# quantumjot/sequitr

Measured on AMD Instinct MI355X. Metric: segmented Mpixels/sec on 512x512 tiles; IoU vs reference, higher is better.
Workload: dtype f32; 1 GPU; U-Net 2-class inference, launches of 32 512x512x1 tiles, fp32 (BASELINE.json configs[1]: filters 16-32-64-128-256, eltwise_mul bridge); logits + uint8 argmax mask; one 32-tile batch per GPU per step; tiles_this_rank=32

## Files before the change

sequitr_amd/csrc/sq_common.h:

```cpp
#pragma once
#include <hip/hip_runtime.h>
#include <stdint.h>
#include <stdio.h>
#include "../../include/sequitr_hip.h"

typedef float f32x4 __attribute__((ext_vector_type(4)));

#define SQ_NOT_MINE 1

void sq_set_error(const char *fmt, ...);

#define SQ_REQUIRE(cond, ...)            \
    do {                                 \
        if (!(cond)) {                   \
            sq_set_error(__VA_ARGS__);   \
            return SQ_EINVAL;            \
        }                                \
    } while (0)

int sq_plan_bf16_kc(int Cin);
int sq_plan_bf16_bn(int64_t ntiles, int Cout, bool pn, bool mos);
int sq_plan_mosaic_splitk(int Nimg, int h, int w, int Cin, int Cout, int R, int Cc, bool have_ws, int64_t workspace_bytes);
int sq_plan_f32_bn(int64_t ntiles, int Cout);
bool sq_plan_f32_stage32(int bn, int KS, int KC, int Cin, bool concat);
bool sq_plan_l0_takes(int mode, int cout, int act, int H, int W, bool concat, int head_c, bool pooled);
int sq_wgrad_f32_plan(int N, int H, int W, int Cin, int Cout, int K, int64_t *out);

#define SQ_ALIGNED16(p) ((((uintptr_t)(p)) & 15u) == 0)

#define SQ_REQUIRE_ALIGNED(p)                                     \
    do {                                                          \
        if (!SQ_ALIGNED16(p)) {                                   \
            sq_set_error("%s: pointer %s not 16-byte aligned", __func__, #p); \
            return SQ_EALIGN;                                     \
        }                                                         \
    } while (0)

static inline int sq_check_launch(const char *what) {
    hipError_t e = hipGetLastError();
    if (e != hipSuccess) {
        sq_set_error("%s: launch failed: %s", what, hipGetErrorString(e));
        return SQ_ELAUNCH;
    }
    return SQ_OK;
}

__device__ __forceinline__ float sq_act(float v, int act) {
    if (act == SQ_ACT_RELU) return v > 0.0f ? v : 0.0f;
    if (act == SQ_ACT_LEAKY) return v > 0.0f ? v : 0.2f * v;
    return v;
}

__device__ __forceinline__ unsigned sq_xcd_remap(unsigned bid, unsigned nblk) {
    const unsigned q = nblk >> 3, r = nblk & 7u, xcd = bid & 7u, k = bid >> 3;
    const unsigned base = xcd < r ? xcd * (q + 1) : r * (q + 1) + (xcd - r) * q;
    return base + k;
}

struct SqDropKey { unsigned s1, s2; };
__device__ __forceinline__ SqDropKey sq_dropout_key(unsigned seed, const int *__restrict__ step) {
    if (step) seed += (unsigned)step[0] * 0x9E3779B9u;
    SqDropKey k;
    k.s1 = seed * 0x9E3779B1u + 0x7F4A7C15u;
    k.s2 = (seed ^ 0x68E31DA4u) * 0x85EBCA6Bu;
    k.s2 ^= k.s2 >> 13;
    return k;
}
__device__ __forceinline__ unsigned sq_dropout_thr16(float rate) { return (unsigned)(rate * 65536.0f); }
__device__ __forceinline__ unsigned sq_dropout_keep4(SqDropKey k, unsigned q, unsigned thr16) {
    unsigned h = q + k.s1;
    h ^= h >> 16; h *= 0x7FEB352Du; h = h ^ (h >> 15) ^ k.s2; h *= 0x846CA68Bu; h ^= h >> 16;
    unsigned g = (h ^ 0x5BD1E995u) * 0x2C1B3C6Du;
    g ^= g >> 15;
    return (unsigned)((h & 0xFFFFu) >= thr16) | ((unsigned)((h >> 16) >= thr16) << 1) |
           ((unsigned)((g & 0xFFFFu) >= thr16) << 2) | ((unsigned)((g >> 16) >= thr16) << 3);
}

template <int MAXC>
__device__ __forceinline__ float sq_wce_pixel(const float (&zc)[MAXC], const float (&yc)[MAXC], int C, float wp, float g,
                                              float *__restrict__ dz) {
#pragma clang fp contract(off)
    float m = -INFINITY, yt = 0.f, dot = 0.f;
#pragma unroll
    for (int c = 0; c < MAXC; ++c)
        if (c < C) {
            m = zc[c] > m ? zc[c] : m;
            yt += yc[c];
            dot = __builtin_fmaf(yc[c], zc[c], dot);
        }
    float s = 0.f;
#pragma unroll
    for (int c = 0; c < MAXC; ++c)
        if (c < C) s += expf(zc[c] - m);
    const float lse = m + logf(s);
    if (dz) {
#pragma unroll
        for (int c = 0; c < MAXC; ++c)
            if (c < C) dz[c] = g * (expf(zc[c] - lse) * yt - yc[c]);
    }
    return wp * (lse * yt - dot);
}

__device__ __forceinline__ float sq_group_reduce(const float *__restrict__ p, size_t stride, int nblk, int g, int G) {
    float s = 0.f;
    int b = g;
    for (; b + 7 * G < nblk; b += 8 * G) {
        float v[8];
#pragma unroll
        for (int u = 0; u < 8; ++u) v[u] = p[(size_t)(b + u * G) * stride];
#pragma unroll
        for (int u = 0; u < 8; ++u) s += v[u];
    }
    for (; b < nblk; b += G) s += p[(size_t)b * stride];
    for (int m = G >> 1; m > 0; m >>= 1) s += __shfl_xor(s, m);
    return s;
}
static inline int sq_group_size(int nblk) {
    int G = 1;
    while (G < 64 && G * 2 <= nblk) G *= 2;
    return G;
}
```

sequitr_amd/csrc/sq_conv_f32_l0.hip:

```cpp
#include <stdlib.h>
#include "sq_common.h"
#include "sq_conv_epi.h"

#ifndef SQ_L0_SETPRIO
#define SQ_L0_SETPRIO 1
#endif
#ifndef SQ_L0_OCC
#define SQ_L0_OCC 4
#endif
#ifndef SQ_L0_UP_OCC
#define SQ_L0_UP_OCC 2
#endif

namespace {

constexpr int TH = 16, TW = 16, HWD = 18, HP = HWD * HWD;
constexpr int PS = 24;
constexpr int XS_FLOATS = HP * PS;
constexpr int XITEMS = HP * 4, XSLOTS = 6;
constexpr int IN_W = 20, IN_FLOATS = IN_W * IN_W;
constexpr int UP_W = 10, UP_CIN = 32, UP_PS = 40, UP_FLOATS = UP_W * UP_W * UP_PS;
constexpr unsigned OOB = 0x80000000u;

enum { EPI_STORE = 0, EPI_POOL = 1, EPI_HEAD = 2 };
enum { M_PLAIN = 0, M_FIRST = 1, M_UP = 2 };

struct L0Args {
    const float *x, *w, *bias;
    float *y;
    int N, H, W;
    int tiles_x, tiles_y, ntiles;
    int gx, gy, gn;
    SqConvEpi epi;
};

struct Pos { int tx, ty, n; };

typedef unsigned u32x4 __attribute__((__vector_size__(4 * sizeof(unsigned))));
typedef unsigned u32x2 __attribute__((__vector_size__(2 * sizeof(unsigned))));

__device__ __forceinline__ void row_transpose(float &a0, float &a1, float &a2, float &a3) {
    const auto p = __builtin_amdgcn_permlane16_swap(__float_as_uint(a0), __float_as_uint(a1), false, false);
    const auto q = __builtin_amdgcn_permlane16_swap(__float_as_uint(a2), __float_as_uint(a3), false, false);
    const auto u = __builtin_amdgcn_permlane32_swap(p[0], q[0], false, false);
    const auto v = __builtin_amdgcn_permlane32_swap(p[1], q[1], false, false);
    a0 = __uint_as_float(u[0]); a2 = __uint_as_float(u[1]);
    a1 = __uint_as_float(v[0]); a3 = __uint_as_float(v[1]);
}

__device__ __forceinline__ float relu(float v) { return __builtin_fmaxf(v, 0.0f); }

template <int MODE, int EPI, int BRIDGE, int NB>
__global__ __launch_bounds__(256, (MODE == M_UP ? SQ_L0_UP_OCC : (NB == 2 ? 2 : SQ_L0_OCC))) void conv_l0_kernel(const L0Args a) {
    static_assert(NB == 1 || (NB == 2 && MODE == M_PLAIN && EPI == EPI_STORE), "32 output channels: the plain form only");
    constexpr int CO = 16 * NB;
    extern __shared__ __attribute__((aligned(16))) float smem[];
    float *xs = smem;
    float *xin = smem + XS_FLOATS;
    float *xl = smem + XS_FLOATS;

    const int tid = threadIdx.x, lane = tid & 63, wv = tid >> 6;
    const int li = lane & 15, kk = lane >> 4;
    const int H = a.H, W = a.W;
    const int G = (int)gridDim.x;
    const int vb = (int)sq_xcd_remap(blockIdx.x, gridDim.x);
    if (vb >= a.ntiles) return;
    const int t_count = (a.ntiles - vb + G - 1) / G;

    const __amdgpu_buffer_rsrc_t xrsrc = __builtin_amdgcn_make_buffer_rsrc(
        const_cast<float *>(a.x), 0, (int)((size_t)a.N * H * W * (MODE == M_FIRST ? 1 : 16) * 4), 0x00020000);
    const __amdgpu_buffer_rsrc_t yrsrc = __builtin_amdgcn_make_buffer_rsrc(
        a.y, 0, a.y ? (int)((size_t)a.N * H * W * CO * 4) : 0, 0x00020000);

    float af[9][4][NB];
#pragma unroll
    for (int t = 0; t < 9; ++t)
#pragma unroll
        for (int s = 0; s < 4; ++s)
#pragma unroll
            for (int nb = 0; nb < NB; ++nb) af[t][s][nb] = a.w[(t * 16 + 4 * s + kk) * CO + nb * 16 + li];
    float4 bv[NB];
#pragma unroll
    for (int nb = 0; nb < NB; ++nb)
        bv[nb] = a.bias ? *reinterpret_cast<const float4 *>(a.bias + nb * 16 + 4 * kk) : make_float4(0.f, 0.f, 0.f, 0.f);

    auto decode = [&](int tile) {
        Pos p;
        p.tx = tile % a.tiles_x;
        p.ty = (tile / a.tiles_x) % a.tiles_y;
        p.n = tile / (a.tiles_x * a.tiles_y);
        return p;
    };
    auto advance = [&](Pos p) {
        p.tx += a.gx;
        if (p.tx >= a.tiles_x) { p.tx -= a.tiles_x; p.ty += 1; }
        p.ty += a.gy;
        if (p.ty >= a.tiles_y) { p.ty -= a.tiles_y; p.n += 1; }
        p.n += a.gn;
        return p;
    };
    auto interior = [&](const Pos &p) {
        return p.tx > 0 && p.tx < a.tiles_x - 1 && p.ty > 0 && p.ty < a.tiles_y - 1;
    };

    float4 xr[XSLOTS];
    int xrel[XSLOTS], xpp[XSLOTS];
    if constexpr (MODE == M_PLAIN) {
#pragma unroll
        for (int sl = 0; sl < XSLOTS; ++sl) {
            const int idx = tid + sl * 256, pix = idx >> 2, q = idx & 3;
            const int py = pix / HWD, px = pix % HWD;
            xrel[sl] = idx < XITEMS ? ((py * W + px) * 16 + q * 4) * 4 : (int)OOB;
            xpp[sl] = (py << 8) | px;
        }
    }
    auto issue_halo = [&](const Pos &p) {
        const int x0 = p.tx * TW - 1, y0 = p.ty * TH - 1;
        const int base = (((p.n * H + y0) * W + x0) * 16) * 4;
        if (interior(p)) {
#pragma unroll
            for (int sl = 0; sl < XSLOTS; ++sl) {
                const auto v = __builtin_amdgcn_raw_buffer_load_b128(xrsrc, xrel[sl], base, 0);
                xr[sl] = *reinterpret_cast<const float4 *>(&v);
            }
        } else {
#pragma unroll
            for (int sl = 0; sl < XSLOTS; ++sl) {
                const int py = xpp[sl] >> 8, px = xpp[sl] & 255;
                const bool inb = (unsigned)(y0 + py) < (unsigned)H && (unsigned)(x0 + px) < (unsigned)W && xrel[sl] != (int)OOB;
                const unsigned off = inb ? (unsigned)(base + xrel[sl]) : OOB;
                const auto v = __builtin_amdgcn_raw_buffer_load_b128(xrsrc, off, 0, 0);
                xr[sl] = *reinterpret_cast<const float4 *>(&v);
            }
        }
    };
    float *cw = xs + (tid >> 2) * PS + (tid & 3);
    auto commit_halo = [&]() {
#pragma unroll
        for (int sl = 0; sl < XSLOTS; ++sl) {
            if (sl < XSLOTS - 1 || tid < XITEMS - (XSLOTS - 1) * 256) {
                float *d = cw + sl * 64 * PS;
                d[0] = xr[sl].x; d[4] = xr[sl].y; d[8] = xr[sl].z; d[12] = xr[sl].w;
            }
        }
    };

    float a1[3] = {0.f, 0.f, 0.f};
    int toff[3] = {0, 0, 0};
    float4 b1v = make_float4(0.f, 0.f, 0.f, 0.f);
    float inr[2] = {0.f, 0.f};
    int fsrc[6] = {0, 0, 0, 0, 0, 0}, fpix[6] = {0, 0, 0, 0, 0, 0};
    int irel[2] = {0, 0};
    if constexpr (MODE == M_FIRST) {
#pragma unroll
        for (int s = 0; s < 3; ++s) {
            const int tap = 4 * s + kk;
            a1[s] = tap < 9 ? a.epi.first_w[tap * 16 + li] : 0.f;
            const int tc = tap < 9 ? tap : 8;
            toff[s] = (tc / 3) * IN_W + tc % 3;
        }
        b1v = *reinterpret_cast<const float4 *>(a.epi.first_b + 4 * kk);
#pragma unroll
        for (int i = 0; i < 6; ++i) {
            const int pix = (wv + 4 * i) * 16 + li, pc = pix < HP ? pix : HP - 1;
            fsrc[i] = (pc / HWD) * IN_W + pc % HWD;
            fpix[i] = pix;
        }
#pragma unroll
        for (int sl = 0; sl < 2; ++sl) {
            const int idx = tid + sl * 256;
            irel[sl] = idx < IN_FLOATS ? ((idx / IN_W) * W + idx % IN_W) * 4 : (int)OOB;
        }
    }
    auto issue_patch = [&](const Pos &p) {
        const int x0 = p.tx * TW - 2, y0 = p.ty * TH - 2;
        const int base = ((p.n * H + y0) * W + x0) * 4;
        if (interior(p)) {
#pragma unroll
            for (int sl = 0; sl < 2; ++sl)
                inr[sl] = __builtin_bit_cast(float, __builtin_amdgcn_raw_buffer_load_b32(xrsrc, irel[sl], base, 0));
        } else {
#pragma unroll
            for (int sl = 0; sl < 2; ++sl) {
                const int idx = tid + sl * 256, py = idx / IN_W, px = idx % IN_W;
                const bool inb = idx < IN_FLOATS && (unsigned)(y0 + py) < (unsigned)H && (unsigned)(x0 + px) < (unsigned)W;
                const unsigned off = inb ? (unsigned)(base + irel[sl]) : OOB;
                inr[sl] = __builtin_bit_cast(float, __builtin_amdgcn_raw_buffer_load_b32(xrsrc, off, 0, 0));
            }
        }
    };
    auto commit_patch = [&](int buf) {
        float *d = xin + buf * IN_FLOATS;
        d[tid] = inr[0];
        if (tid < IN_FLOATS - 256) d[tid + 256] = inr[1];
    };
    auto first_conv = [&](const Pos &p, int buf) {
        const float *src = xin + buf * IN_FLOATS;
        const bool inner = interior(p);
#pragma unroll
        for (int i = 0; i < 6; ++i) {
            if (wv + 4 * i < (HP + 15) / 16) {
                f32x4 c1 = (f32x4){0.f, 0.f, 0.f, 0.f};
#pragma unroll
                for (int s = 0; s < 3; ++s)
                    c1 = __builtin_amdgcn_mfma_f32_16x16x4f32(a1[s], src[fsrc[i] + toff[s]], c1, 0, 0, 0);
                float v0 = relu(c1[0] + b1v.x), v1 = relu(c1[1] + b1v.y), v2 = relu(c1[2] + b1v.z), v3 = relu(c1[3] + b1v.w);
                if (!inner) {
                    const int pc = fpix[i] < HP ? fpix[i] : HP - 1;
                    const int gy = p.ty * TH - 1 + pc / HWD, gx = p.tx * TW - 1 + pc % HWD;
                    const bool inside = (unsigned)gy < (unsigned)H && (unsigned)gx < (unsigned)W;
                    v0 = inside ? v0 : 0.f; v1 = inside ? v1 : 0.f; v2 = inside ? v2 : 0.f; v3 = inside ? v3 : 0.f;
                }
                row_transpose(v0, v1, v2, v3);
                if (fpix[i] < HP) *reinterpret_cast<float4 *>(xs + fpix[i] * PS + 4 * kk) = make_float4(v0, v1, v2, v3);
            }
        }
    };

    float aw[8] = {0.f, 0.f, 0.f, 0.f, 0.f, 0.f, 0.f, 0.f};
    float4 upb = make_float4(0.f, 0.f, 0.f, 0.f);
    float4 lr[4], sr[6];
    int srel[6] = {0, 0, 0, 0, 0, 0}, lrel[4] = {0, 0, 0, 0};
    unsigned upk[6] = {0, 0, 0, 0, 0, 0};
    const int Hl = H >> 1, Wl = W >> 1;
    const __amdgpu_buffer_rsrc_t lrsrc = __builtin_amdgcn_make_buffer_rsrc(
        const_cast<float *>(a.epi.up_x), 0, MODE == M_UP ? (int)((size_t)a.N * Hl * Wl * UP_CIN * 4) : 0, 0x00020000);
    if constexpr (MODE == M_UP) {
#pragma unroll
        for (int s8 = 0; s8 < 8; ++s8) aw[s8] = a.epi.up_w[(wv * 16 + li) * UP_CIN + 4 * s8 + kk];
        if (a.epi.up_b) upb = *reinterpret_cast<const float4 *>(a.epi.up_b + 4 * kk);
        const int oy = ((wv >> 1) + 1) & 1, ox = ((wv & 1) + 1) & 1;
#pragma unroll
        for (int blk = 0; blk < 6; ++blk) {
            const int j = blk * 16 + li, jc = j < 81 ? j : 80;
            const int hy = 2 * (jc / 9) + oy, hx = 2 * (jc % 9) + ox;
            srel[blk] = j < 81 ? ((hy * W + hx) * 16 + 4 * kk) * 4 : (int)OOB;
            const unsigned usrc = (((hy + 1) >> 1) * UP_W + ((hx + 1) >> 1)) * UP_PS + 4 * kk;
            const unsigned udst = j < 81 ? (hy * HWD + hx) * PS + 4 * kk : 0xFFFFu;
            upk[blk] = usrc | (udst << 16);
        }
#pragma unroll
        for (int sl = 0; sl < 4; ++sl) {
            const int idx = tid + sl * 256, lp = idx >> 3, q = idx & 7;
            lrel[sl] = idx < UP_W * UP_W * 8 ? (((lp / UP_W) * Wl + lp % UP_W) * UP_CIN + q * 4) * 4 : (int)OOB;
        }
    }
    auto issue_skip = [&](const Pos &p) {
        const int x0 = p.tx * TW - 1, y0 = p.ty * TH - 1;
        const int base = (((p.n * H + y0) * W + x0) * 16) * 4;
        if (interior(p)) {
#pragma unroll
            for (int blk = 0; blk < 6; ++blk) {
                const auto v = __builtin_amdgcn_raw_buffer_load_b128(xrsrc, srel[blk], base, 0);
                sr[blk] = *reinterpret_cast<const float4 *>(&v);
            }
        } else {
            const int oy = ((wv >> 1) + 1) & 1, ox = ((wv & 1) + 1) & 1;
#pragma unroll
            for (int blk = 0; blk < 6; ++blk) {
                const int j = blk * 16 + li, jc = j < 81 ? j : 80;
                const int hy = 2 * (jc / 9) + oy, hx = 2 * (jc % 9) + ox;
                const bool inb = j < 81 && (unsigned)(y0 + hy) < (unsigned)H && (unsigned)(x0 + hx) < (unsigned)W;
                const unsigned off = inb ? (unsigned)(base + srel[blk]) : OOB;
                const auto v = __builtin_amdgcn_raw_buffer_load_b128(xrsrc, off, 0, 0);
                sr[blk] = *reinterpret_cast<const float4 *>(&v);
            }
        }
    };
    auto issue_low = [&](const Pos &p) {
        const int ly0 = p.ty * (TH / 2) - 1, lx0 = p.tx * (TW / 2) - 1;
        const int base = (((p.n * Hl + ly0) * Wl + lx0) * UP_CIN) * 4;
        if (interior(p)) {
#pragma unroll
            for (int sl = 0; sl < 4; ++sl) {
                const auto v = __builtin_amdgcn_raw_buffer_load_b128(lrsrc, lrel[sl], base, 0);
                lr[sl] = *reinterpret_cast<const float4 *>(&v);
            }
        } else {
#pragma unroll
            for (int sl = 0; sl < 4; ++sl) {
                const int idx = tid + sl * 256, lp = idx >> 3;
                const int ly = lp / UP_W, lx = lp % UP_W;
                const bool inb = idx < UP_W * UP_W * 8 && (unsigned)(ly0 + ly) < (unsigned)Hl && (unsigned)(lx0 + lx) < (unsigned)Wl;
                const unsigned off = inb ? (unsigned)(base + lrel[sl]) : OOB;
                const auto v = __builtin_amdgcn_raw_buffer_load_b128(lrsrc, off, 0, 0);
                lr[sl] = *reinterpret_cast<const float4 *>(&v);
            }
        }
    };
    float *lw = xl + (tid >> 3) * UP_PS + ((tid & 7) >> 2) * 16 + (tid & 3);
    auto commit_low = [&]() {
#pragma unroll
        for (int sl = 0; sl < 4; ++sl) {
            if (sl < 3 || tid < UP_W * UP_W * 8 - 768) {
                float *d = lw + sl * 32 * UP_PS;
                d[0] = lr[sl].x; d[4] = lr[sl].y; d[8] = lr[sl].z; d[12] = lr[sl].w;
            }
        }
    };
    auto up_conv = [&](const Pos &p) {
        const bool inner = interior(p);
#pragma unroll
        for (int bp = 0; bp < 6; bp += 2) {
            float4 bl[2][2];
#pragma unroll
            for (int t = 0; t < 2; ++t) {
                const float *src = xl + (upk[bp + t] & 0xFFFFu);
                bl[t][0] = *reinterpret_cast<const float4 *>(src);
                bl[t][1] = *reinterpret_cast<const float4 *>(src + 16);
            }
            f32x4 c1[2];
#pragma unroll
            for (int s8 = 0; s8 < 8; ++s8) {
#pragma unroll
                for (int t = 0; t < 2; ++t) {
                    const float4 q = bl[t][s8 >> 2];
                    const float b = (s8 & 3) == 0 ? q.x : ((s8 & 3) == 1 ? q.y : ((s8 & 3) == 2 ? q.z : q.w));
                    c1[t] = __builtin_amdgcn_mfma_f32_16x16x4f32(aw[s8], b, s8 == 0 ? (f32x4){0.f, 0.f, 0.f, 0.f} : c1[t], 0, 0, 0);
                }
            }
#pragma unroll
            for (int t = 0; t < 2; ++t) {
                const int blk = bp + t;
                const float u[4] = {c1[t][0] + upb.x, c1[t][1] + upb.y, c1[t][2] + upb.z, c1[t][3] + upb.w};
                const float sk[4] = {sr[blk].x, sr[blk].y, sr[blk].z, sr[blk].w};
                float m[4];
#pragma unroll
                for (int e = 0; e < 4; ++e)
                    m[e] = BRIDGE == SQ_BRIDGE_ADD ? u[e] + sk[e]
                         : (BRIDGE == SQ_BRIDGE_MUL ? u[e] * sk[e] : (BRIDGE == SQ_BRIDGE_SUB ? u[e] - sk[e] : u[e]));
                if (!inner) {
                    const int j = blk * 16 + li, jc = j < 81 ? j : 80;
                    const int hy = 2 * (jc / 9) + (((wv >> 1) + 1) & 1), hx = 2 * (jc % 9) + (((wv & 1) + 1) & 1);
                    const int gy = p.ty * TH - 1 + hy, gx = p.tx * TW - 1 + hx;
                    const bool inside = (unsigned)gy < (unsigned)H && (unsigned)gx < (unsigned)W;
#pragma unroll
                    for (int e = 0; e < 4; ++e) m[e] = inside ? m[e] : 0.f;
                }
                row_transpose(m[0], m[1], m[2], m[3]);
                if ((upk[blk] >> 16) != 0xFFFFu) *reinterpret_cast<float4 *>(xs + (upk[blk] >> 16)) = make_float4(m[0], m[1], m[2], m[3]);
            }
        }
    };

    f32x4 acc[4][NB];
    const float *xb = xs + ((4 * wv) * HWD + li) * PS + 4 * kk;
    auto mfma_phase = [&]() {
        float4 bq[2][3];
#pragma unroll
        for (int kx = 0; kx < 3; ++kx) bq[0][kx] = *reinterpret_cast<const float4 *>(xb + kx * PS);
#if SQ_L0_SETPRIO
        __builtin_amdgcn_s_setprio(0);
#endif
#pragma unroll
        for (int h = 0; h < 6; ++h) {
            if (h + 1 < 6) {
#pragma unroll
                for (int kx = 0; kx < 3; ++kx)
                    bq[(h + 1) & 1][kx] = *reinterpret_cast<const float4 *>(xb + ((h + 1) * HWD + kx) * PS);
            }
            __builtin_amdgcn_sched_barrier(0);
#pragma unroll
            for (int kx = 0; kx < 3; ++kx) {
                const float4 q = bq[h & 1][kx];
                const float b[4] = {q.x, q.y, q.z, q.w};
#pragma unroll
                for (int s = 0; s < 4; ++s) {
#pragma unroll
                    for (int ky = 2; ky >= 0; --ky) {
                        const int r = h - ky;
                        if (r < 0 || r > 3) continue;
                        const bool first = ky == 0 && kx == 0 && s == 0;
#pragma unroll
                        for (int nb = 0; nb < NB; ++nb)
                            acc[r][nb] = __builtin_amdgcn_mfma_f32_16x16x4f32(af[ky * 3 + kx][s][nb], b[s],
                                                                              first ? (f32x4){0.f, 0.f, 0.f, 0.f} : acc[r][nb], 0, 0, 0);
                    }
                }
            }
            __builtin_amdgcn_sched_barrier(0);
        }
#if SQ_L0_SETPRIO
        __builtin_amdgcn_s_setprio(3);
#endif
    };

    const int yvoff = (((4 * wv) * W + li) * CO + 4 * kk) * 4;
    const __amdgpu_buffer_rsrc_t prsrc = __builtin_amdgcn_make_buffer_rsrc(
        a.epi.pooled, 0, EPI == EPI_POOL ? (int)((size_t)a.N * Hl * Wl * 16 * 4) : 0, 0x00020000);
    const int pvoff = (((2 * wv) * Wl + (li >> 1)) * 16 + 4 * kk) * 4;
    float *hws = smem + XS_FLOATS;
    float hb0 = 0.f, hb1 = 0.f;
    const __amdgpu_buffer_rsrc_t grsrc = __builtin_amdgcn_make_buffer_rsrc(
        a.epi.logits, 0, EPI == EPI_HEAD ? (int)((size_t)a.N * H * W * 2 * 4) : 0, 0x00020000);
    const __amdgpu_buffer_rsrc_t mrsrc = __builtin_amdgcn_make_buffer_rsrc(
        a.epi.mask, 0, (EPI == EPI_HEAD && a.epi.mask) ? (int)((size_t)a.N * H * W) : 0, 0x00020000);
    const int gvoff = ((4 * wv + kk) * W + li) * 8, mvoff = (4 * wv + kk) * W + li;
    if constexpr (EPI == EPI_HEAD) {
        static_assert(MODE == M_PLAIN, "the head table sits right behind the halo image");
        if (tid < 64) hws[tid] = (tid >> 4) < 2 ? a.epi.head_w[(tid & 15) * 2 + (tid >> 4)] : 0.f;
        if (a.epi.head_b) { hb0 = a.epi.head_b[0]; hb1 = a.epi.head_b[1]; }
    }
    auto epilogue = [&](const Pos &p) {
        if constexpr (NB > 1) {
            const int tbase = (((p.n * H + p.ty * TH) * W + p.tx * TW) * CO) * 4;
#pragma unroll
            for (int r = 0; r < 4; ++r)
#pragma unroll
                for (int nb = 0; nb < NB; ++nb) {
                    const f32x4 t = (f32x4){relu(acc[r][nb][0] + bv[nb].x), relu(acc[r][nb][1] + bv[nb].y),
                                            relu(acc[r][nb][2] + bv[nb].z), relu(acc[r][nb][3] + bv[nb].w)};
                    __builtin_amdgcn_raw_buffer_store_b128(*reinterpret_cast<const u32x4 *>(&t), yrsrc,
                                                           yvoff + tbase + r * W * CO * 4 + nb * 64, 0, 0);
                }
            return;
        }
        float o[4][4];
#pragma unroll
        for (int r = 0; r < 4; ++r) {
            o[r][0] = relu(acc[r][0][0] + bv[0].x); o[r][1] = relu(acc[r][0][1] + bv[0].y);
            o[r][2] = relu(acc[r][0][2] + bv[0].z); o[r][3] = relu(acc[r][0][3] + bv[0].w);
        }
        if constexpr (EPI != EPI_HEAD) {
            const int tbase = (((p.n * H + p.ty * TH) * W + p.tx * TW) * 16) * 4;
#pragma unroll
            for (int r = 0; r < 4; ++r) {
                const f32x4 t = (f32x4){o[r][0], o[r][1], o[r][2], o[r][3]};
                __builtin_amdgcn_raw_buffer_store_b128(*reinterpret_cast<const u32x4 *>(&t), yrsrc, yvoff + tbase + r * W * 64, 0, 0);
            }
        }
        if constexpr (EPI == EPI_POOL) {
            const int pbase = (((p.n * Hl + p.ty * (TH / 2)) * Wl + p.tx * (TW / 2)) * 16) * 4;
#pragma unroll
            for (int pr = 0; pr < 2; ++pr) {
                f32x4 mp;
#pragma unroll
                for (int j = 0; j < 4; ++j) {
                    const float v = __builtin_fmaxf(o[2 * pr][j], o[2 * pr + 1][j]);
                    const float u = __builtin_bit_cast(float, __builtin_amdgcn_mov_dpp(__builtin_bit_cast(int, v), 0xB1, 0xF, 0xF, true));
                    mp[j] = __builtin_fmaxf(u, v);
                }
                __builtin_amdgcn_raw_buffer_store_b128(*reinterpret_cast<const u32x4 *>(&mp), prsrc,
                                                       (li & 1) ? (int)OOB : pvoff + pbase + pr * Wl * 64, 0, 0);
            }
        }
        if constexpr (EPI == EPI_HEAD) {
#pragma unroll
            for (int j = 0; j < 4; ++j) row_transpose(o[0][j], o[1][j], o[2][j], o[3][j]);
            float4 hq[4];
#pragma unroll
            for (int r = 0; r < 4; ++r) hq[r] = *reinterpret_cast<const float4 *>(hws + (lane & 3) * 16 + 4 * r);
            f32x4 z = (f32x4){0.f, 0.f, 0.f, 0.f};
#pragma unroll
            for (int r = 0; r < 4; ++r) {
                const float hv[4] = {hq[r].x, hq[r].y, hq[r].z, hq[r].w};
#pragma unroll
                for (int j = 0; j < 4; ++j) z = __builtin_amdgcn_mfma_f32_4x4x1f32(hv[j], o[r][j], z, 0, 0, 0);
            }
            const float z0 = z[0], z1 = z[1];
            const float v0 = a.epi.head_b ? z0 + hb0 : z0, v1 = a.epi.head_b ? z1 + hb1 : z1;
            const int pbase = (p.n * H + p.ty * TH) * W + p.tx * TW;
            const float lg[2] = {v0, v1};
            __builtin_amdgcn_raw_buffer_store_b64(*reinterpret_cast<const u32x2 *>(lg), grsrc, gvoff, pbase * 8, 0);
            __builtin_amdgcn_raw_buffer_store_b8((unsigned char)(v1 > v0 ? 1 : 0), mrsrc, mvoff, pbase, 0);
        }
    };

    Pos cur = decode(vb), nxt = cur, nn = cur;
    if constexpr (MODE == M_PLAIN) {
        issue_halo(cur);
        __builtin_amdgcn_s_waitcnt(0x0F70);
        commit_halo();
        __syncthreads();
        for (int it = 0; it < t_count; ++it) {
            const bool has_next = it + 1 < t_count;
            if (has_next) { nxt = advance(cur); issue_halo(nxt); }
            mfma_phase();
            __builtin_amdgcn_s_waitcnt(0x0F70);
            if (has_next) {
                __syncthreads();
                commit_halo();
            }
            epilogue(cur);
            if (has_next) __syncthreads();
            cur = nxt;
        }
    }
    if constexpr (MODE == M_FIRST) {
        issue_patch(cur);
        __builtin_amdgcn_s_waitcnt(0x0F70);
        commit_patch(0);
        __syncthreads();
        first_conv(cur, 0);
        if (t_count > 1) {
            nxt = advance(cur);
            issue_patch(nxt);
            __builtin_amdgcn_s_waitcnt(0x0F70);
            commit_patch(1);
        }
        __syncthreads();
        for (int it = 0; it < t_count; ++it) {
            const bool has_next = it + 1 < t_count, has_next2 = it + 2 < t_count;
            if (has_next2) { nn = advance(nxt); issue_patch(nn); }
            mfma_phase();
            __builtin_amdgcn_s_waitcnt(0x0F70);
            if (has_next) {
                __syncthreads();
                first_conv(nxt, (it + 1) & 1);
            }
            if (has_next2) commit_patch(it & 1);
            epilogue(cur);
            if (has_next) __syncthreads();
            cur = nxt;
            nxt = nn;
        }
    }
    if constexpr (MODE == M_UP) {
        issue_low(cur);
        issue_skip(cur);
        __builtin_amdgcn_s_waitcnt(0x0F70);
        commit_low();
        if (t_count > 1) { nxt = advance(cur); issue_low(nxt); }
        __syncthreads();
        up_conv(cur);
        __builtin_amdgcn_s_waitcnt(0x0F70);
        __syncthreads();
        for (int it = 0; it < t_count; ++it) {
            const bool has_next = it + 1 < t_count, has_next2 = it + 2 < t_count;
            if (has_next) { commit_low(); issue_skip(nxt); }
            if (has_next2) { nn = advance(nxt); issue_low(nn); }
            mfma_phase();
            __builtin_amdgcn_s_waitcnt(0x0F70);
            if (has_next) {
                __syncthreads();
                up_conv(nxt);
            }
            epilogue(cur);
            if (has_next) __syncthreads();
            cur = nxt;
            nxt = nn;
        }
    }
}

template <int MODE, int EPI, int BRIDGE = 0, int NB = 1>
int launch_l0(const L0Args &a0, hipStream_t st) {
    static bool attr_set = false;
    auto kern = conv_l0_kernel<MODE, EPI, BRIDGE, NB>;
    constexpr int lds = (XS_FLOATS + (MODE == M_FIRST ? 2 * IN_FLOATS : (MODE == M_UP ? UP_FLOATS : 0)) + (EPI == EPI_HEAD ? 64 : 0)) * 4;
    if (!attr_set) {
        if (hipFuncSetAttribute(reinterpret_cast<const void *>(kern), hipFuncAttributeMaxDynamicSharedMemorySize, lds) != hipSuccess) {
            sq_set_error("conv_l0: cannot reserve %d bytes of LDS", lds);
            return SQ_ELAUNCH;
        }
        attr_set = true;
    }
    L0Args a = a0;
    a.tiles_x = a.W / TW;
    a.tiles_y = a.H / TH;
    a.ntiles = a.tiles_x * a.tiles_y * a.N;
    const int want = 256 * (MODE == M_UP ? SQ_L0_UP_OCC : (NB == 2 ? 2 : SQ_L0_OCC));
    const int G = a.ntiles < want ? a.ntiles : want;
    const int per_image = a.tiles_x * a.tiles_y;
    a.gn = G / per_image;
    a.gy = (G % per_image) / a.tiles_x;
    a.gx = (G % per_image) % a.tiles_x;
    hipLaunchKernelGGL(kern, dim3(G), dim3(256), lds, st, a);
    return sq_check_launch("conv_l0");
}

}

int sq_conv_l0_launch(int mode, const float *x, const float *w, const float *bias, float *y, int N, int H, int W,
                      int cout, int act, const SqConvEpi &epi, hipStream_t st) {
    if (!sq_plan_l0_takes(mode, cout, act, H, W, epi.x2 != nullptr, epi.head_w ? epi.head_c : 0,
                          epi.pooled != nullptr))
        return SQ_L0_NOT_MINE;
    L0Args a = {};
    a.x = x; a.w = w; a.bias = bias; a.y = y; a.N = N; a.H = H; a.W = W; a.epi = epi;
    const int e = epi.head_w ? EPI_HEAD : (epi.pooled ? EPI_POOL : EPI_STORE);
    if (mode == M_PLAIN) {
        if (e == EPI_HEAD) return launch_l0<M_PLAIN, EPI_HEAD>(a, st);
        if (e == EPI_POOL) return launch_l0<M_PLAIN, EPI_POOL>(a, st);
        if (cout == 32) return launch_l0<M_PLAIN, EPI_STORE, 0, 2>(a, st);
        return launch_l0<M_PLAIN, EPI_STORE>(a, st);
    }
    if (mode == M_FIRST) {
        if (e == EPI_HEAD) return SQ_L0_NOT_MINE;
        if (e == EPI_POOL) return launch_l0<M_FIRST, EPI_POOL>(a, st);
        return launch_l0<M_FIRST, EPI_STORE>(a, st);
    }
    if (mode == M_UP) {
        if (e != EPI_STORE) return SQ_L0_NOT_MINE;
        switch (epi.up_bridge) {
            case SQ_BRIDGE_ADD: return launch_l0<M_UP, EPI_STORE, SQ_BRIDGE_ADD>(a, st);
            case SQ_BRIDGE_MUL: return launch_l0<M_UP, EPI_STORE, SQ_BRIDGE_MUL>(a, st);
            case SQ_BRIDGE_SUB: return launch_l0<M_UP, EPI_STORE, SQ_BRIDGE_SUB>(a, st);
            default: return launch_l0<M_UP, EPI_STORE, SQ_BRIDGE_NONE>(a, st);
        }
    }
    return SQ_L0_NOT_MINE;
}
```

sequitr_amd/csrc/sq_convt_loss.hip:

```cpp
#include <stdlib.h>
#include "sq_common.h"

namespace {

template <int KCH>
__global__ __launch_bounds__(256) void convT2x2_mfma_f32_kernel(
    const float *__restrict__ x, const float *__restrict__ w, const float *__restrict__ bias,
    const float *__restrict__ skip, float *__restrict__ y, int64_t P, int H, int W, int Cin,
    int Cout, int bridge) {
    constexpr int CT_PS = KCH + 2;
    __shared__ __attribute__((aligned(16))) float as[64 * CT_PS];
    __shared__ __attribute__((aligned(16))) float xs[64 * CT_PS];
    const int tid = threadIdx.x, lane = tid & 63, wv = tid >> 6;
    const int li = lane & 15, kk = lane >> 4;
    const int64_t p0 = (int64_t)blockIdx.x * 64;
    const int r0 = blockIdx.y * 64;

    const int rho = r0 + 16 * wv + 4 * kk;
    const bool row_ok = rho < 4 * Cout;
    const int ab = row_ok ? rho / Cout : 0, o = row_ok ? rho % Cout : 0;
    const int pa = ab >> 1, pb = ab & 1;
    size_t off[4];
    bool ok[4];
    float4 sk[4];
    int64_t nn;
    int ii, jj;
    {
        const int64_t pl = p0 + li < P ? p0 + li : 0;
        if (P < ((int64_t)1 << 31)) {
            const unsigned pu = (unsigned)pl, t = pu / (unsigned)W;
            jj = (int)(pu - t * (unsigned)W);
            const unsigned n32 = t / (unsigned)H;
            ii = (int)(t - n32 * (unsigned)H);
            nn = n32;
        } else {
            jj = (int)(pl % W);
            const int64_t t = pl / W;
            ii = (int)(t % H);
            nn = t / H;
        }
    }
#pragma unroll
    for (int cb = 0; cb < 4; ++cb) {
        const int64_t p = p0 + cb * 16 + li;
        ok[cb] = row_ok && p < P;
        off[cb] = ((size_t)(nn * 2 * H + 2 * ii + pa) * (2 * W) + 2 * jj + pb) * Cout + o;
        sk[cb] = make_float4(0.f, 0.f, 0.f, 0.f);
        if (bridge != SQ_BRIDGE_NONE && ok[cb]) sk[cb] = *reinterpret_cast<const float4 *>(skip + off[cb]);
        jj += 16;
        while (jj >= W) {
            jj -= W;
            if (++ii == H) { ii = 0; ++nn; }
        }
    }

    float4 bv = make_float4(0.f, 0.f, 0.f, 0.f);
    if (bias && row_ok) bv = *reinterpret_cast<const float4 *>(bias + o);

    f32x4 acc[4];
#pragma unroll
    for (int cb = 0; cb < 4; ++cb) acc[cb] = (f32x4){0.f, 0.f, 0.f, 0.f};

    constexpr int QPR = KCH / 4;
    constexpr int NIT = QPR / 4;
    float4 vr[NIT], ur[NIT];
    auto issue = [&](int cc) {
#pragma unroll
        for (int it = 0; it < NIT; ++it) {
            const int idx = tid + it * 256, srow = idx / QPR, sq = idx % QPR;
            vr[it] = make_float4(0.f, 0.f, 0.f, 0.f);
            ur[it] = make_float4(0.f, 0.f, 0.f, 0.f);
            if (r0 + srow < 4 * Cout)
                vr[it] = *reinterpret_cast<const float4 *>(w + (size_t)(r0 + srow) * Cin + cc + sq * 4);
            if (p0 + srow < P)
                ur[it] = *reinterpret_cast<const float4 *>(x + (size_t)(p0 + srow) * Cin + cc + sq * 4);
        }
    };
    auto commit = [&]() {
#pragma unroll
        for (int it = 0; it < NIT; ++it) {
            const int idx = tid + it * 256, srow = idx / QPR, sq = idx % QPR;
            float *d = as + srow * CT_PS + sq * 4;
            *reinterpret_cast<float2 *>(d) = make_float2(vr[it].x, vr[it].y);
            *reinterpret_cast<float2 *>(d + 2) = make_float2(vr[it].z, vr[it].w);
            float *e = xs + srow * CT_PS + sq * 4;
            *reinterpret_cast<float2 *>(e) = make_float2(ur[it].x, ur[it].y);
            *reinterpret_cast<float2 *>(e + 2) = make_float2(ur[it].z, ur[it].w);
        }
    };
    issue(0);
    for (int cc = 0; cc < Cin; cc += KCH) {
        commit();
        __syncthreads();
        if (cc + KCH < Cin) issue(cc + KCH);
#pragma unroll 4
        for (int s = 0; s < QPR; ++s) {
            const float a = as[(16 * wv + li) * CT_PS + s * 4 + kk];
            float b[4];
#pragma unroll
            for (int cb = 0; cb < 4; ++cb) b[cb] = xs[(cb * 16 + li) * CT_PS + s * 4 + kk];
#pragma unroll
            for (int cb = 0; cb < 4; ++cb)
                acc[cb] = __builtin_amdgcn_mfma_f32_16x16x4f32(a, b[cb], acc[cb], 0, 0, 0);
        }
        __syncthreads();
    }

    if (!row_ok) return;
#pragma unroll
    for (int cb = 0; cb < 4; ++cb) {
        if (!ok[cb]) continue;
        float4 v = make_float4(acc[cb][0] + bv.x, acc[cb][1] + bv.y, acc[cb][2] + bv.z, acc[cb][3] + bv.w);
        if (!bias) v = make_float4(acc[cb][0], acc[cb][1], acc[cb][2], acc[cb][3]);
        if (bridge != SQ_BRIDGE_NONE) {
            const float4 k = sk[cb];
            if (bridge == SQ_BRIDGE_ADD) v = make_float4(v.x + k.x, v.y + k.y, v.z + k.z, v.w + k.w);
            else if (bridge == SQ_BRIDGE_MUL) v = make_float4(v.x * k.x, v.y * k.y, v.z * k.z, v.w * k.w);
            else v = make_float4(v.x - k.x, v.y - k.y, v.z - k.z, v.w - k.w);
        }
        *reinterpret_cast<float4 *>(y + off[cb]) = v;
    }
}

constexpr int CE_MAXC = 8;

__global__ __launch_bounds__(256) void wsoftmax_ce_f32_kernel(
    const float *__restrict__ z, const uint8_t *__restrict__ yoh, const float *__restrict__ wgt,
    int64_t npix, int C, float gscale, double *__restrict__ partials, float *__restrict__ dz) {
    __shared__ double red[256];
    double tsum = 0.0;
    for (int64_t p = (int64_t)blockIdx.x * 256 + threadIdx.x; p < npix; p += (int64_t)gridDim.x * 256) {
        float zc[CE_MAXC], yc[CE_MAXC], dzc[CE_MAXC];
#pragma unroll
        for (int c = 0; c < CE_MAXC; ++c) {
            zc[c] = yc[c] = 0.f;
            if (c < C) {
                zc[c] = z[p * C + c];
                yc[c] = (float)yoh[p * C + c];
            }
        }
        const float wp = wgt[p];
        tsum += (double)sq_wce_pixel<CE_MAXC>(zc, yc, C, wp, wp * gscale, dz ? dzc : nullptr);
        if (dz) {
#pragma unroll
            for (int c = 0; c < CE_MAXC; ++c)
                if (c < C) dz[p * C + c] = dzc[c];
        }
    }
    red[threadIdx.x] = tsum;
    __syncthreads();
    for (int s = 128; s > 0; s >>= 1) {
        if ((int)threadIdx.x < s) red[threadIdx.x] += red[threadIdx.x + s];
        __syncthreads();
    }
    if (threadIdx.x == 0) partials[blockIdx.x] = red[0];
}

__global__ __launch_bounds__(256) void ce_finish_kernel(const double *__restrict__ partials, int n, double inv_npix,
                                                        double *__restrict__ loss) {
    __shared__ double red[256];
    double s = 0.0;
    for (int i = threadIdx.x; i < n; i += 256) s += partials[i];
    red[threadIdx.x] = s;
    __syncthreads();
    for (int k = 128; k > 0; k >>= 1) {
        if ((int)threadIdx.x < k) red[threadIdx.x] += red[threadIdx.x + k];
        __syncthreads();
    }
    if (threadIdx.x == 0) *loss = red[0] * inv_npix;
}

inline int64_t ce_blocks(int64_t npix) {
    int64_t b = (npix + 255) / 256;
    return b > 2048 ? 2048 : (b < 1 ? 1 : b);
}

}

int sq_convT_v2_launch(const float *x, const float *w, const float *bias, const float *skip, float *y, int N, int H,
                       int W, int Cin, int Cout, int bridge, hipStream_t st);

extern "C" int sq_convT2x2s2_nhwc_fwd_f32(const float *x, const float *w, const float *bias,
                                          const float *skip, float *y, int N, int H, int W, int Cin,
                                          int Cout, int bridge, void *stream) {
    SQ_REQUIRE(x && w && y, "sq_convT2x2s2_nhwc_fwd_f32: null tensor pointer");
    SQ_REQUIRE(N > 0 && H > 0 && W > 0, "sq_convT2x2s2_nhwc_fwd_f32: bad shape");
    SQ_REQUIRE(Cin % 16 == 0 && Cout % 4 == 0 && Cin > 0 && Cout > 0,
               "sq_convT2x2s2_nhwc_fwd_f32: Cin=%d must be a multiple of 16, Cout=%d of 4", Cin, Cout);
    SQ_REQUIRE(bridge >= SQ_BRIDGE_NONE && bridge <= SQ_BRIDGE_SUB, "sq_convT2x2s2_nhwc_fwd_f32: bad bridge %d", bridge);
    SQ_REQUIRE(bridge == SQ_BRIDGE_NONE || skip, "sq_convT2x2s2_nhwc_fwd_f32: bridge needs a skip tensor");
    SQ_REQUIRE_ALIGNED(x); SQ_REQUIRE_ALIGNED(w); SQ_REQUIRE_ALIGNED(y);
    if (bias) SQ_REQUIRE_ALIGNED(bias);
    if (skip) SQ_REQUIRE_ALIGNED(skip);
    {
        const int r = sq_convT_v2_launch(x, w, bias, skip, y, N, H, W, Cin, Cout, bridge, reinterpret_cast<hipStream_t>(stream));
        if (r != SQ_NOT_MINE) return r;
    }
    const int64_t P = (int64_t)N * H * W;
    dim3 grid((unsigned)((P + 63) / 64), (unsigned)((4 * Cout + 63) / 64));
    static const int kch = [] { const char *e = getenv("SQ_CONVT_KCH"); return e ? atoi(e) : 32; }();
    if (Cin % 32 == 0 && kch == 32)
        hipLaunchKernelGGL(convT2x2_mfma_f32_kernel<32>, grid, dim3(256), 0, reinterpret_cast<hipStream_t>(stream),
                           x, w, bias, skip, y, P, H, W, Cin, Cout, bridge);
    else
        hipLaunchKernelGGL(convT2x2_mfma_f32_kernel<16>, grid, dim3(256), 0, reinterpret_cast<hipStream_t>(stream),
                           x, w, bias, skip, y, P, H, W, Cin, Cout, bridge);
    return sq_check_launch("sq_convT2x2s2_nhwc_fwd_f32");
}

extern "C" int64_t sq_wsoftmax_ce_partials(int64_t npix) { return npix > 0 ? ce_blocks(npix) : 0; }

extern "C" int sq_wsoftmax_ce_fwd_bwd_f32(const float *logits, const uint8_t *onehot,
                                          const float *weights, int64_t npix, int C, float grad_scale,
                                          double *partials, double *loss, float *dlogits, void *stream) {
    SQ_REQUIRE(logits && onehot && weights && partials && loss, "sq_wsoftmax_ce_fwd_bwd_f32: null pointer");
    SQ_REQUIRE(npix > 0 && C >= 1 && C <= CE_MAXC, "sq_wsoftmax_ce_fwd_bwd_f32: C=%d unsupported (1..%d)", C, CE_MAXC);
    hipStream_t st = reinterpret_cast<hipStream_t>(stream);
    const int nb = (int)ce_blocks(npix);
    hipLaunchKernelGGL(wsoftmax_ce_f32_kernel, dim3(nb), dim3(256), 0, st, logits, onehot, weights, npix, C,
                       grad_scale / (float)npix, partials, dlogits);
    int rc = sq_check_launch("sq_wsoftmax_ce_fwd_bwd_f32");
    if (rc) return rc;
    hipLaunchKernelGGL(ce_finish_kernel, dim3(1), dim3(256), 0, st, partials, nb, 1.0 / (double)npix, loss);
    return sq_check_launch("sq_wsoftmax_ce_fwd_bwd_f32(finish)");
}
```

Measured before the change: 1648 Mpixels/s.

## Add persistent weight-stationary streaming transposed-conv kernel with register-held weights

Adds a new persistent 2x2 stride-2 transposed convolution kernel that keeps each wave's weight rows in registers and streams pixel groups through MFMA. It double-buffers input loads with buffer intrinsics so the next chunk is fetched while the current one is multiplied, and remaps blocks across XCDs. The bias/bridge epilogue is fused into the output store. This targets the LDS staging and repeated weight reloads of the previous convT path, at the cost of high register pressure and a separate code path that falls back to the old kernel for unsupported shapes. The row-transpose helper moves into the shared header.

```diff
diff --git a/sequitr_amd/csrc/sq_common.h b/sequitr_amd/csrc/sq_common.h
--- a/sequitr_amd/csrc/sq_common.h
+++ b/sequitr_amd/csrc/sq_common.h
@@ -55,6 +55,15 @@
     const unsigned q = nblk >> 3, r = nblk & 7u, xcd = bid & 7u, k = bid >> 3;
     const unsigned base = xcd < r ? xcd * (q + 1) : r * (q + 1) + (xcd - r) * q;
     return base + k;
+}
+
+__device__ __forceinline__ void sq_row_transpose(float &a0, float &a1, float &a2, float &a3) {
+    const auto p = __builtin_amdgcn_permlane16_swap(__float_as_uint(a0), __float_as_uint(a1), false, false);
+    const auto q = __builtin_amdgcn_permlane16_swap(__float_as_uint(a2), __float_as_uint(a3), false, false);
+    const auto u = __builtin_amdgcn_permlane32_swap(p[0], q[0], false, false);
+    const auto v = __builtin_amdgcn_permlane32_swap(p[1], q[1], false, false);
+    a0 = __uint_as_float(u[0]); a2 = __uint_as_float(u[1]);
+    a1 = __uint_as_float(v[0]); a3 = __uint_as_float(v[1]);
 }
 
 struct SqDropKey { unsigned s1, s2; };
diff --git a/sequitr_amd/csrc/sq_conv_f32_l0.hip b/sequitr_amd/csrc/sq_conv_f32_l0.hip
--- a/sequitr_amd/csrc/sq_conv_f32_l0.hip
+++ b/sequitr_amd/csrc/sq_conv_f32_l0.hip
@@ -39,15 +39,6 @@
 typedef unsigned u32x4 __attribute__((__vector_size__(4 * sizeof(unsigned))));
 typedef unsigned u32x2 __attribute__((__vector_size__(2 * sizeof(unsigned))));
 
-__device__ __forceinline__ void row_transpose(float &a0, float &a1, float &a2, float &a3) {
-    const auto p = __builtin_amdgcn_permlane16_swap(__float_as_uint(a0), __float_as_uint(a1), false, false);
-    const auto q = __builtin_amdgcn_permlane16_swap(__float_as_uint(a2), __float_as_uint(a3), false, false);
-    const auto u = __builtin_amdgcn_permlane32_swap(p[0], q[0], false, false);
-    const auto v = __builtin_amdgcn_permlane32_swap(p[1], q[1], false, false);
-    a0 = __uint_as_float(u[0]); a2 = __uint_as_float(u[1]);
-    a1 = __uint_as_float(v[0]); a3 = __uint_as_float(v[1]);
-}
-
 __device__ __forceinline__ float relu(float v) { return __builtin_fmaxf(v, 0.0f); }
 
 template <int MODE, int EPI, int BRIDGE, int NB>
@@ -211,7 +202,7 @@
                     const bool inside = (unsigned)gy < (unsigned)H && (unsigned)gx < (unsigned)W;
                     v0 = inside ? v0 : 0.f; v1 = inside ? v1 : 0.f; v2 = inside ? v2 : 0.f; v3 = inside ? v3 : 0.f;
                 }
-                row_transpose(v0, v1, v2, v3);
+                sq_row_transpose(v0, v1, v2, v3);
                 if (fpix[i] < HP) *reinterpret_cast<float4 *>(xs + fpix[i] * PS + 4 * kk) = make_float4(v0, v1, v2, v3);
             }
         }
@@ -337,7 +328,7 @@
 #pragma unroll
                     for (int e = 0; e < 4; ++e) m[e] = inside ? m[e] : 0.f;
                 }
-                row_transpose(m[0], m[1], m[2], m[3]);
+                sq_row_transpose(m[0], m[1], m[2], m[3]);
                 if ((upk[blk] >> 16) != 0xFFFFu) *reinterpret_cast<float4 *>(xs + (upk[blk] >> 16)) = make_float4(m[0], m[1], m[2], m[3]);
             }
         }
@@ -446,7 +437,7 @@
         }
         if constexpr (EPI == EPI_HEAD) {
 #pragma unroll
-            for (int j = 0; j < 4; ++j) row_transpose(o[0][j], o[1][j], o[2][j], o[3][j]);
+            for (int j = 0; j < 4; ++j) sq_row_transpose(o[0][j], o[1][j], o[2][j], o[3][j]);
             float4 hq[4];
 #pragma unroll
             for (int r = 0; r < 4; ++r) hq[r] = *reinterpret_cast<const float4 *>(hws + (lane & 3) * 16 + 4 * r);
diff --git a/sequitr_amd/csrc/sq_convt_f32_stream.hip b/sequitr_amd/csrc/sq_convt_f32_stream.hip
--- /dev/null
+++ b/sequitr_amd/csrc/sq_convt_f32_stream.hip
@@ -0,0 +1,192 @@
+#include <stdlib.h>
+#include <type_traits>
+#include "sq_common.h"
+
+namespace {
+
+constexpr unsigned OOB = 0x80000000u;
+
+typedef unsigned u32x4 __attribute__((__vector_size__(4 * sizeof(unsigned))));
+
+struct CsArgs {
+    const float *x, *w, *bias, *skip;
+    float *y;
+    int P, H, W, Cout;
+    int nsq, ngroups;
+};
+
+template <int CIN, int RB, int KC, int OCC, int BRIDGE>
+__global__ __launch_bounds__(256, OCC) void convT2x2_stream_kernel(const CsArgs a) {
+    constexpr int NCH = CIN / KC, QC = KC / 16, NQ = CIN / 16;
+    static_assert(CIN % KC == 0 && KC % 16 == 0, "whole chunks of whole float4 quads");
+    const int tid = threadIdx.x, lane = tid & 63, wv = tid >> 6;
+    const int li = lane & 15, kk = lane >> 4;
+    const int Cout = a.Cout, H = a.H, W = a.W, P = a.P;
+    const int G = (int)gridDim.x;
+    const int vb = (int)sq_xcd_remap(blockIdx.x, gridDim.x);
+    const int gs = G / a.nsq;
+    const int g0 = vb / a.nsq;
+    if (g0 >= a.ngroups) return;
+    const int cnt = (a.ngroups - g0 + gs - 1) / gs;
+    const int row0 = ((vb % a.nsq) * 4 + wv) * 16 * RB;
+
+    const __amdgpu_buffer_rsrc_t xrsrc = __builtin_amdgcn_make_buffer_rsrc(
+        const_cast<float *>(a.x), 0, (int)((size_t)P * CIN * 4), 0x00020000);
+    const int out_bytes = (int)((size_t)P * 4 * Cout * 4);
+    const __amdgpu_buffer_rsrc_t srsrc = __builtin_amdgcn_make_buffer_rsrc(
+        const_cast<float *>(a.skip), 0, BRIDGE != SQ_BRIDGE_NONE ? out_bytes : 0, 0x00020000);
+    const __amdgpu_buffer_rsrc_t yrsrc = __builtin_amdgcn_make_buffer_rsrc(a.y, 0, out_bytes, 0x00020000);
+
+    float af[RB][CIN / 4];
+    int clsoff[RB], boff[RB];
+    float4 bq[RB];
+#pragma unroll
+    for (int rb = 0; rb < RB; ++rb) {
+        const float *wr = a.w + (size_t)(row0 + 16 * rb + li) * CIN + 4 * kk;
+#pragma unroll
+        for (int q = 0; q < NQ; ++q) {
+            float4 v = *reinterpret_cast<const float4 *>(wr + 16 * q);
+            sq_row_transpose(v.x, v.y, v.z, v.w);
+            af[rb][4 * q + 0] = v.x; af[rb][4 * q + 1] = v.y; af[rb][4 * q + 2] = v.z; af[rb][4 * q + 3] = v.w;
+        }
+        const int rho = row0 + 16 * rb + 4 * kk;
+        const int ab = rho / Cout, o = rho - ab * Cout;
+        clsoff[rb] = (((ab >> 1) * 2 * W + (ab & 1)) * Cout + o) * 4;
+        boff[rb] = o;
+    }
+
+    const int step_px = gs * 16;
+    const int s_j = step_px % W, s_i = (step_px / W) % H, s_n = step_px / (W * H);
+    unsigned gp = (unsigned)g0 * 16u + (unsigned)li;
+    int gj, gi, gn;
+    {
+        const unsigned pu = gp < (unsigned)P ? gp : 0u, t = pu / (unsigned)W;
+        gj = (int)(pu - t * (unsigned)W);
+        gn = (int)(t / (unsigned)H);
+        gi = (int)(t - (unsigned)gn * (unsigned)H);
+    }
+    auto xoffset = [&](unsigned p, bool live) {
+        return (live && p < (unsigned)P) ? (p * (unsigned)CIN + 4u * (unsigned)kk) * 4u : OOB;
+    };
+
+    float4 xb[2][QC];
+    auto issue_x = [&](float4 (&dst)[QC], unsigned off, int chunk) {
+#pragma unroll
+        for (int q = 0; q < QC; ++q) {
+            const auto v = __builtin_amdgcn_raw_buffer_load_b128(xrsrc, off + (unsigned)((chunk * KC + 16 * q) * 4), 0, 0);
+            dst[q] = *reinterpret_cast<const float4 *>(&v);
+        }
+    };
+
+    f32x4 acc[RB];
+    float4 sk[RB];
+    int it = 0;
+    auto do_group = [&](auto parc) {
+        constexpr int PAR = decltype(parc)::value;
+        const unsigned pixoff = gp < (unsigned)P ? (unsigned)((((gn * 2 * H + 2 * gi) * (2 * W)) + 2 * gj) * Cout * 4) : OOB;
+        const unsigned xcur = xoffset(gp, true), xnext = xoffset(gp + (unsigned)step_px, it + 1 < cnt);
+        if constexpr (BRIDGE != SQ_BRIDGE_NONE) {
+#pragma unroll
+            for (int rb = 0; rb < RB; ++rb) {
+                const auto v = __builtin_amdgcn_raw_buffer_load_b128(srsrc, pixoff == OOB ? OOB : pixoff + (unsigned)clsoff[rb], 0, 0);
+                sk[rb] = *reinterpret_cast<const float4 *>(&v);
+            }
+        }
+#pragma unroll
+        for (int c = 0; c < NCH; ++c) {
+            float4 (&cur)[QC] = xb[(PAR + c) & 1];
+            if (c + 1 < NCH) issue_x(xb[(PAR + c + 1) & 1], xcur, c + 1);
+            else issue_x(xb[(PAR + c + 1) & 1], xnext, 0);
+            __builtin_amdgcn_s_setprio(0);
+            __builtin_amdgcn_sched_barrier(0);
+#pragma unroll
+            for (int q = 0; q < QC; ++q) {
+                float4 v = cur[q];
+                sq_row_transpose(v.x, v.y, v.z, v.w);
+                const float b[4] = {v.x, v.y, v.z, v.w};
+#pragma unroll
+                for (int s = 0; s < 4; ++s)
+#pragma unroll
+                    for (int rb = 0; rb < RB; ++rb)
+                        acc[rb] = __builtin_amdgcn_mfma_f32_16x16x4f32(
+                            af[rb][(c * QC + q) * 4 + s], b[s],
+                            (c == 0 && q == 0 && s == 0) ? (f32x4){0.f, 0.f, 0.f, 0.f} : acc[rb], 0, 0, 0);
+            }
+            __builtin_amdgcn_sched_barrier(0);
+            __builtin_amdgcn_s_setprio(3);
+        }
+#pragma unroll
+        for (int rb = 0; rb < RB; ++rb) {
+            f32x4 v = acc[rb];
+            if (a.bias) { v[0] += bq[rb].x; v[1] += bq[rb].y; v[2] += bq[rb].z; v[3] += bq[rb].w; }
+            if constexpr (BRIDGE == SQ_BRIDGE_ADD) { v[0] += sk[rb].x; v[1] += sk[rb].y; v[2] += sk[rb].z; v[3] += sk[rb].w; }
+            if constexpr (BRIDGE == SQ_BRIDGE_MUL) { v[0] *= sk[rb].x; v[1] *= sk[rb].y; v[2] *= sk[rb].z; v[3] *= sk[rb].w; }
+            if constexpr (BRIDGE == SQ_BRIDGE_SUB) { v[0] -= sk[rb].x; v[1] -= sk[rb].y; v[2] -= sk[rb].z; v[3] -= sk[rb].w; }
+            __builtin_amdgcn_raw_buffer_store_b128(*reinterpret_cast<const u32x4 *>(&v), yrsrc,
+                                                   pixoff == OOB ? OOB : pixoff + (unsigned)clsoff[rb], 0, 0);
+        }
+        gp += (unsigned)step_px;
+        gj += s_j;
+        if (gj >= W) { gj -= W; gi += 1; }
+        gi += s_i;
+        if (gi >= H) { gi -= H; gn += 1; }
+        gn += s_n;
+        ++it;
+    };
+
+    issue_x(xb[0], xoffset(gp, true), 0);
+    __builtin_amdgcn_sched_barrier(0);
+#pragma unroll
+    for (int rb = 0; rb < RB; ++rb) bq[rb] = *reinterpret_cast<const float4 *>((a.bias ? a.bias : a.w) + boff[rb]);
+    __builtin_amdgcn_sched_barrier(0);
+    while (it < cnt) {
+        do_group(std::integral_constant<int, 0>{});
+        if constexpr (NCH & 1) {
+            if (it < cnt) do_group(std::integral_constant<int, 1>{});
+        }
+    }
+}
+
+template <int CIN, int RB, int KC, int OCC, int BRIDGE>
+int launch_one(const CsArgs &a0, hipStream_t st) {
+    CsArgs a = a0;
+    a.nsq = a.Cout / 4 / RB / 4;
+    a.ngroups = (a.P + 15) / 16;
+    const long total = (long)a.nsq * a.ngroups;
+    const int want = 256 * OCC;
+    int G = total < want ? (int)total : want;
+    if (G > a.nsq) G -= G % a.nsq;
+    hipLaunchKernelGGL((convT2x2_stream_kernel<CIN, RB, KC, OCC, BRIDGE>), dim3(G), dim3(256), 0, st, a);
+    return sq_check_launch("sq_convT2x2s2_nhwc_fwd_f32(stream)");
+}
+
+template <int CIN, int RB, int KC, int OCC>
+int launch_cs(const CsArgs &a, int bridge, hipStream_t st) {
+    switch (bridge) {
+        case SQ_BRIDGE_ADD: return launch_one<CIN, RB, KC, OCC, SQ_BRIDGE_ADD>(a, st);
+        case SQ_BRIDGE_MUL: return launch_one<CIN, RB, KC, OCC, SQ_BRIDGE_MUL>(a, st);
+        case SQ_BRIDGE_SUB: return launch_one<CIN, RB, KC, OCC, SQ_BRIDGE_SUB>(a, st);
+        default: return launch_one<CIN, RB, KC, OCC, SQ_BRIDGE_NONE>(a, st);
+    }
+}
+
+}
+
+int sq_convT_stream_launch(const float *x, const float *w, const float *bias, const float *skip, float *y, int N, int H,
+                           int W, int Cin, int Cout, int bridge, hipStream_t st) {
+    static const bool off = [] { const char *e = getenv("SQ_CONVT_V3"); return e && e[0] == '0'; }();
+    if (off) return SQ_NOT_MINE;
+    const size_t P = (size_t)N * H * W;
+    if (Cout % 32 != 0) return SQ_NOT_MINE;
+    if (P * 4 * Cout * 4 >= ((size_t)1 << 31) || P * Cin * 4 >= ((size_t)1 << 31)) return SQ_NOT_MINE;
+    CsArgs a = {};
+    a.x = x; a.w = w; a.bias = bias; a.skip = skip; a.y = y;
+    a.P = (int)P; a.H = H; a.W = W; a.Cout = Cout;
+    switch (Cin) {
+        case 32: return launch_cs<32, 2, 32, 4>(a, bridge, st);
+        case 64: return launch_cs<64, 2, 64, 4>(a, bridge, st);
+        case 128: return launch_cs<128, 2, 64, 3>(a, bridge, st);
+        case 256: return launch_cs<256, 2, 64, 2>(a, bridge, st);
+        default: return SQ_NOT_MINE;
+    }
+}
diff --git a/sequitr_amd/csrc/sq_convt_loss.hip b/sequitr_amd/csrc/sq_convt_loss.hip
--- a/sequitr_amd/csrc/sq_convt_loss.hip
+++ b/sequitr_amd/csrc/sq_convt_loss.hip
@@ -179,6 +179,8 @@
 
 int sq_convT_v2_launch(const float *x, const float *w, const float *bias, const float *skip, float *y, int N, int H,
                        int W, int Cin, int Cout, int bridge, hipStream_t st);
+int sq_convT_stream_launch(const float *x, const float *w, const float *bias, const float *skip, float *y, int N, int H,
+                           int W, int Cin, int Cout, int bridge, hipStream_t st);
 
 extern "C" int sq_convT2x2s2_nhwc_fwd_f32(const float *x, const float *w, const float *bias,
                                           const float *skip, float *y, int N, int H, int W, int Cin,
@@ -193,7 +195,9 @@
     if (bias) SQ_REQUIRE_ALIGNED(bias);
     if (skip) SQ_REQUIRE_ALIGNED(skip);
     {
-        const int r = sq_convT_v2_launch(x, w, bias, skip, y, N, H, W, Cin, Cout, bridge, reinterpret_cast<hipStream_t>(stream));
+        int r = sq_convT_stream_launch(x, w, bias, skip, y, N, H, W, Cin, Cout, bridge, reinterpret_cast<hipStream_t>(stream));
+        if (r != SQ_NOT_MINE) return r;
+        r = sq_convT_v2_launch(x, w, bias, skip, y, N, H, W, Cin, Cout, bridge, reinterpret_cast<hipStream_t>(stream));
         if (r != SQ_NOT_MINE) return r;
     }
     const int64_t P = (int64_t)N * H * W;
```

Result: no change. 1639 Mpixels/s (-0.5%).
